# bioinfo-biols/CIRI-long

Measured on AMD Instinct MI355X. Metric: reads/s through CCS+SSW+BSJ (1/2/4/8 MI355X); % HBM roofline, higher is better.
Workload: dtype int16

## Files before the change

ciri_long_amd/csrc/ccs_poa.hip:

```cpp
#include <hip/hip_runtime.h>
#include <stdint.h>
#include "clh_device.h"
#include "clh_device_ops.h"

namespace clh {

static constexpr int CCS_K = 8;
static constexpr int CCS_DMIN = 30;
static constexpr int CCS_MIN_SUPPORT = 12;
static constexpr int CCS_SMOOTH = 3;
static constexpr int CCS_MAX_CUTS = 64;
static constexpr int CCS_MIN_TAIL = 20;
static constexpr int CCS_GUARD = 8;
static constexpr int POA_MAXP = 12;
static constexpr int POA_MAXP_ALL = 48;
static constexpr int POA_OVF_CAP = 2048;
static constexpr int POA_MAXA = 7;
static constexpr int POA_MAX_COPY = 2800;

__device__ __forceinline__ void phase_sync() {
    __syncthreads();
#ifdef POA_AGENT_PHASE_SYNC
    __builtin_amdgcn_fence(__ATOMIC_ACQUIRE, "agent");
#else
// ... 385 lines not shown
    for (int t = 1; t < CP; ++t) { runA[t] = pk_max(runA[t - 1], a[t - 1]); runB[t] = pk_max(runB[t - 1], b[t - 1]); }
    const uint32_t totA = pk_max(runA[CP - 1], a[CP - 1]), totB = pk_max(runB[CP - 1], b[CP - 1]);
    const int loA = (int)(short)(totA & 0xffffu), hiA = (int)totA >> 16, loB = (int)(short)(totB & 0xffffu), hiB = (int)totB >> 16;
    int excA = dpp_shr1(leftA, loA > hiA ? loA : hiA), excB = dpp_shr1(leftB, loB > hiB ? loB : hiB);
    wave_prefix_max2(excA, excB);
    const uint32_t exA = pack_exc(excA, totA), exB = pack_exc(excB, totB);
#pragma unroll
    for (int t = 0; t < CP; ++t) { pa[t] = pk_max(runA[t], exA); pb[t] = pk_max(runB[t], exB); }
}

__device__ __forceinline__ uint32_t pk_nz_select(uint32_t x, uint32_t d, uint32_t lo) {
    uint32_t r;
    asm("v_pk_min_u16 %0, %1, 1 op_sel_hi:[1,0]\n\tv_pk_mad_u16 %0, %0, %2, %3" : "=&v"(r) : "v"(x), "v"(d), "v"(lo));
    return r;
}
__device__ __forceinline__ uint32_t lshl_or(uint32_t a, int sh, uint32_t b) {
    uint32_t d;
    asm("v_lshl_or_b32 %0, %1, %2, %3" : "=v"(d) : "v"(a), "n"(sh), "v"(b));
    return d;
}
template <typename T>
__device__ __forceinline__ T* uniform_ptr(T* p) {
    const unsigned long long v = (unsigned long long)p;
    const uint32_t lo = (uint32_t)__builtin_amdgcn_readfirstlane((int)(uint32_t)v), hi = (uint32_t)__builtin_amdgcn_readfirstlane((int)(uint32_t)(v >> 32));
    typedef __attribute__((address_space(1))) T* gptr;
    return (T*)(gptr)(((unsigned long long)hi << 32) | lo);
}

template <int HX, int HY>
__device__ __forceinline__ uint32_t mix16(uint32_t x, uint32_t y) {
// ... 11 lines not shown
__device__ __forceinline__ void to_packed(const uint32_t (&nat)[CP], uint32_t (&p)[CP]) {
    if constexpr (CP == 1) p[0] = nat[0];
    else if constexpr (CP == 2) { p[0] = mix16<0, 0>(nat[0], nat[1]); p[1] = mix16<1, 1>(nat[0], nat[1]); }
    else if constexpr (CP == 3) { p[0] = mix16<0, 1>(nat[0], nat[1]); p[1] = mix16<1, 0>(nat[0], nat[2]); p[2] = mix16<0, 1>(nat[1], nat[2]); }
    else { p[0] = mix16<0, 0>(nat[0], nat[2]); p[1] = mix16<1, 1>(nat[0], nat[2]); p[2] = mix16<0, 0>(nat[1], nat[3]); p[3] = mix16<1, 1>(nat[1], nat[3]); }
}

static constexpr int D_F = 0x0007, D_O_SHIFT = 3, D_E_SHIFT = 8, D_Q_SHIFT = 11;
#ifndef POA_BAND_W
#define POA_BAND_W 32
#endif
static constexpr int POA_BAND = POA_BAND_W;
static constexpr int POA_H_NONE = -32768;
static constexpr int BT_MISS = -2;

template <int CP, bool SIMPLE = false>
__device__ void dp_pass_lz(const PoaWs& w, const PoaScores S, int N, int m, const int8_t* seq, int lane, const int pass, const int colbase,
                           const bool more_in, const int RING, const int slope16, int& bs_io, int& br_io, int& bc_io DBGARG)
{
    constexpr int C = 2 * CP;
    const int gp = poa_pitch(m);
    const int rmask = RING - 1;
    const bool more = SIMPLE ? false : more_in;
    const bool sw = SIMPLE ? true : (S.algorithm & 0xff) == 0, nw = SIMPLE ? false : (S.algorithm & 0xff) == 1;
    char* const gH = (char*)uniform_ptr(w.planeH);
    char* const gD = (char*)uniform_ptr(w.planeD);
    const uint2* const gri = uniform_ptr(w.ri);
    const short* const gcol0 = uniform_ptr(w.col0);
    const int cpitch = __builtin_amdgcn_readfirstlane(w.cpitch);
    const int32_t* const gorder = uniform_ptr(w.order); const int32_t* const grank = uniform_ptr(w.rank); const int32_t* const gpred = uniform_ptr(w.pred);
    const int g = S.g, e = S.e, q = S.q, c = S.c;
    const uint32_t g2 = dup16(g), e2 = dup16(e), q2 = dup16(q), c2 = dup16(c);
    const uint32_t sm2 = opaque(dup16(S.m)), dsn2 = opaque(dup16(S.n - S.m));
    const uint32_t ge2 = dup16(g - e), qc2 = dup16(q - c);
    const uint32_t NEG2 = dup16(POA_NEG), ONE2 = 0x00010001u;
    const uint32_t floor2 = sw ? 0u : 0x80008000u;
    const bool beyond_free = sw && S.n < 0 && S.g < 0 && S.q < 0;
    uint32_t* ring = poa_lds;
    const int rrow = 128 * poa_ring_cp(m);
    int* ringL = (int*)(poa_lds + RING * rrow);
    const bool last = !more;
    const int lc0 = C * lane, col0 = colbase + lc0;
    const int mc = m - 1 - colbase;
    const int lm = mc / C, tm = (mc % C) % CP, hm = (mc % C) / CP;
    uint32_t sbP[CP], jeP[CP], jcP[CP];
#pragma unroll
    for (int t = 0; t < CP; ++t) {
        const int jlo = col0 + t + 1, jhi = jlo + CP;
        sbP[t] = pack16(jlo <= m ? (int)(uint8_t)seq[jlo - 1] : 0x100, jhi <= m ? (int)(uint8_t)seq[jhi - 1] : 0x100);
        jeP[t] = pack16((lc0 + t + 1) * e, (lc0 + CP + t + 1) * e);
        jcP[t] = pack16((lc0 + t + 1) * c, (lc0 + CP + t + 1) * c);
    }
    auto row0_h = [&](int j) -> int {
        const int l1 = g + (j - 1) * e, l2 = q + (j - 1) * c;
        return (sw || j == 0) ? 0 : (l1 > l2 ? l1 : l2);
    };
    short* const gcarry = uniform_ptr(w.carry);
    const short* cprev = gcarry + (size_t)(pass & 1) * 3 * cpitch;
    short* cnext = gcarry + (size_t)((pass + 1) & 1) * 3 * cpitch;
    const bool carried = SIMPLE ? false : pass > 0;
    uint2 blk = make_uint2(0, 0); int cH = 0, cE = POA_NEG, cQ = POA_NEG;
    struct RowIn { uint2 b; int h, e, q; };
    auto fetch1 = [&](int rr) -> RowIn {
        const bool in = rr <= N;
        const int rc = in ? rr : N;
        const uint2 b = gri[rc];
        const int hc = (int)cprev[rc], ec = (int)cprev[cpitch + rc], qc = (int)cprev[2 * cpitch + rc], h0 = (int)gcol0[rc];
        RowIn x;
        x.b = in ? b : make_uint2(0, 0);
        x.h = !in ? 0 : (carried ? hc : (nw ? h0 : 0));
        x.e = in && carried ? ec : POA_NEG; x.q = in && carried ? qc : POA_NEG;
        return x;
    };
    auto fetch = [&](int rr, uint2& b, int& h, int& ee, int& qq) { const RowIn x = fetch1(rr); b = x.b; h = x.h; ee = x.e; qq = x.q; };
    auto left_of = [&](int qr) -> int { return carried ? (int)cprev[qr] : (nw ? (int)gcol0[qr] : 0); };
    fetch(1 + lane, blk, cH, cE, cQ);
    asm volatile("" :: "v"(blk.x), "v"(blk.y), "v"(cH), "v"(cE), "v"(cQ));
    uint32_t px[CP], pf[CP], po[CP];
    int pcin = 0;
#pragma unroll
    for (int t = 0; t < CP; ++t) { px[t] = 0; pf[t] = 0; po[t] = 0; }
    uint32_t bsP = sw ? 0u : 0x80008000u, brP = 0;
    uint32_t snapP[CP];
#pragma unroll
    for (int t = 0; t < CP; ++t) snapP[t] = 0;
    int nbest = -(1 << 30), nrow = 0;
    uint32_t lowP = 0x7fff7fffu;
    const bool stores = col0 + 1 <= m;
    const uint32_t lane_off = (uint32_t)(col0 + 8) * 2u;
    uint32_t beyondP[CP], endP[CP];
#pragma unroll
    for (int t = 0; t < CP; ++t) { beyondP[t] = opaque(pk_sra15(sbP[t] << 7)); endP[t] = opaque(beyond_free ? 0u : beyondP[t]); }
    for (int rb = 1; rb <= N; rb += 64) {
        uint2 nblk; int nH, nE, nQ;
        fetch(rb + 64 + lane, nblk, nH, nE, nQ);
        const int cnt = N - rb + 1 < 64 ? N - rb + 1 : 64;
        int cobH = 0, cobE = 0, cobQ = 0;
        for (int i = 0; i < cnt; ++i) {
            const int r = rb + i;
            SEC0();
            const uint32_t d0 = (uint32_t)__builtin_amdgcn_readlane((int)blk.x, i);
            int cinH = 0, cinE = POA_NEG, cinQ = POA_NEG;
            if (__builtin_expect(carried | nw, 0)) cinH = __builtin_amdgcn_readlane(cH, i);
            if (__builtin_expect(carried, 0)) { cinE = __builtin_amdgcn_readlane(cE, i); cinQ = __builtin_amdgcn_readlane(cQ, i); }
            const int vb = (int)(d0 & 0xff), np = (int)((d0 >> 8) & 0xf);
            const bool sink = (d0 & 0x1000u) != 0, tolds = (d0 & 0x4000u) != 0;
            const int p0 = (int)(d0 >> 16);
            uint32_t ss[CP];
            {
                const uint32_t vb2 = dup16(vb);
#pragma unroll
                for (int t = 0; t < CP; ++t) {
                    ss[t] = pk_nz_select(sbP[t] ^ vb2, dsn2, sm2);
                }
            }
            auto source = [&](int qr, uint32_t (&h)[CP], int& left, uint32_t (&fs)[CP], uint32_t (&os)[CP]) {
                if (qr == 0) {
#pragma unroll
                    for (int t = 0; t < CP; ++t) {
                        h[t] = pack16(row0_h(col0 + t + 1), row0_h(col0 + CP + t + 1));
                        fs[t] = pk_adds(h[t], 0xffffffffu); os[t] = fs[t];
                    }
                    left = row0_h(colbase);
                } else {
                    uint32_t dd[CP];
                    if (r - qr < RING) {
                        const uint32_t* rp = ring + (qr & rmask) * rrow + lane * CP;
#pragma unroll
                        for (int t = 0; t < CP; ++t) { h[t] = rp[t]; dd[t] = rp[64 * CP + t]; }
                        left = ringL[qr & rmask];
                    } else {
                        uint32_t nh[CP], nd[CP];
                        const uint32_t* sh = (const uint32_t*)(gH + (size_t)qr * gp * 2 + lane_off);
                        const uint32_t* sd = (const uint32_t*)(gD + (size_t)qr * gp * 2 + lane_off);
#pragma unroll
                        for (int t = 0; t < CP; ++t) {
                            nh[t] = 0; nd[t] = 0;
                            if (stores) {
                                nh[t] = __hip_atomic_load(sh + t, __ATOMIC_RELAXED, __HIP_MEMORY_SCOPE_AGENT);
                                nd[t] = __hip_atomic_load(sd + t, __ATOMIC_RELAXED, __HIP_MEMORY_SCOPE_AGENT);
                            }
                        }
                        left = left_of(qr);
                        to_packed<CP>(nh, h); to_packed<CP>(nd, dd);
                    }
#pragma unroll
                    for (int t = 0; t < CP; ++t) {
                        fs[t] = pk_adds(h[t], pk_subu(dd[t] & 0x00070007u, ONE2));
                        os[t] = pk_adds(h[t], pk_subu(pk_shr(dd[t], 3) & 0x001f001fu, ONE2));
                    }
                }
            };
            SEC(8);
            uint32_t dg[CP], MF[CP], MO[CP];
            auto one_source = [&]() {
                const uint32_t hsh0 = hand_down(px[CP - 1], pcin);
#pragma unroll
                for (int t = 0; t < CP; ++t) {
                    dg[t] = pk_adds(t == 0 ? hsh0 : px[t - 1], ss[t]);
                    MF[t] = pk_max(px[t], pf[t]); MO[t] = pk_max(px[t], po[t]);
                }
            };
            if (__builtin_expect((d0 & 0x2000u) != 0, 1)) {
                one_source();
            } else if (np <= 1) {
                source(np == 0 ? 0 : p0, px, pcin, pf, po);
                one_source();
            } else {
                const uint32_t d1 = (uint32_t)__builtin_amdgcn_readlane((int)blk.y, i);
#pragma unroll
                for (int t = 0; t < CP; ++t) { dg[t] = NEG2; MF[t] = NEG2; MO[t] = NEG2; }
                auto add_source = [&](int qr) {
                    uint32_t h[CP], fs[CP], os[CP];
                    int left = pcin;
                    if (qr == r - 1) {
#pragma unroll
                        for (int t = 0; t < CP; ++t) { h[t] = px[t]; fs[t] = pf[t]; os[t] = po[t]; }
                    } else source(qr, h, left, fs, os);
                    const uint32_t hsh0 = hand_down(h[CP - 1], left);
#pragma unroll
                    for (int t = 0; t < CP; ++t) {
                        dg[t] = pk_max(dg[t], pk_adds(t == 0 ? hsh0 : h[t - 1], ss[t]));
                        MF[t] = pk_max(MF[t], pk_max(h[t], fs[t])); MO[t] = pk_max(MO[t], pk_max(h[t], os[t]));
                    }
                };
                add_source(p0);
                add_source((int)(d1 & 0xffff));
                if (np > 2) add_source((int)(d1 >> 16));
                if (np > 3) {
                    const int vnode = __builtin_amdgcn_readfirstlane(gorder[r - 1]);
                    const int npt = np < 15 ? np : __builtin_amdgcn_readfirstlane((int)w.np[vnode]);
                    for (int s2 = 3; s2 < npt; ++s2) add_source(__builtin_amdgcn_readfirstlane(grank[poa_pred_at(w, vnode, s2)]));
                }
            }
            SEC(9);
            uint32_t M0[CP], fsn[CP], osn[CP];
#pragma unroll
            for (int t = 0; t < CP; ++t) {
                fsn[t] = pk_adds(MF[t], e2); osn[t] = pk_adds(MO[t], c2);
                M0[t] = pk_max(pk_max(dg[t], floor2), pk_max(pk_adds(MF[t], g2), pk_adds(MO[t], q2)));
            }
            uint32_t X[CP], Y[CP];
            {
                uint32_t a[CP], b[CP], pe[CP], pq[CP];
                const int leftE = cinH > cinE + e - g ? cinH : cinE + e - g;
                const int leftQ = cinH > cinQ + c - q ? cinH : cinQ + c - q;
#pragma unroll
                for (int t = 0; t < CP; ++t) { a[t] = pk_subs(M0[t], jeP[t]); b[t] = pk_subs(M0[t], jcP[t]); }
                scan_left_pk2<CP>(a, leftE, pe, b, leftQ, pq);
#pragma unroll
                for (int t = 0; t < CP; ++t) { X[t] = pk_adds(pe[t], jeP[t]); Y[t] = pk_adds(pq[t], jcP[t]); }
            }
            SEC(10);
            uint32_t Hf[CP], qhat[CP], Es[CP], D[CP];
#pragma unroll
            for (int t = 0; t < CP; ++t) { qhat[t] = pk_adds(Y[t], qc2); Hf[t] = pk_max(pk_max(M0[t], pk_adds(X[t], ge2)), qhat[t]); }
            const uint32_t q0 = hand_down(qhat[CP - 1], cinQ);
#pragma unroll
            for (int t = 0; t < CP; ++t) {
                Es[t] = pk_max(X[t], pk_adds(t == 0 ? q0 : qhat[t - 1], e2));
                const uint32_t Hm = pk_subs(Hf[t], ONE2);
                const uint32_t YF = pk_max(fsn[t], Hm), YO = pk_max(osn[t], Hm), YE = pk_max(Es[t], Hm), YQ = pk_max(Y[t], Hm);
                {
                    uint32_t dd_, t_;
                    asm("v_pk_mad_u16 %0, %2, 8, %3 op_sel_hi:[1,0,1]\n\tv_pk_mad_u16 %1, %4, 8, %5 op_sel_hi:[1,0,1]\n\t"
                        "v_pk_mad_u16 %0, %1, %6, %0\n\tv_pk_mad_u16 %0, %7, %8, %0"
                        : "=&v"(dd_), "=&v"(t_) : "v"(YO), "v"(YF), "v"(YQ), "v"(YE), "s"(0x01000100u), "v"(Hm), "s"(dup16(-2313)));
                    D[t] = dd_;
                }
            }
            SEC(11);
#pragma unroll
            for (int t = 0; t < CP; ++t) { px[t] = Hf[t]; pf[t] = fsn[t]; po[t] = osn[t]; }
            pcin = cinH;
            const int band = (slope16 && !(d0 & 0x8000u)) ? POA_BAND : (1 << 20);
            const int cen = (int)(((unsigned)r * (unsigned)slope16) >> 16);
            const bool st_row = stores && (unsigned)(col0 + C - (cen - band)) <= (unsigned)(2 * band + C - 1);
            if (__builtin_expect(st_row, 1)) {
                uint32_t nh[CP], nd[CP];
                to_natural<CP>(Hf, nh); to_natural<CP>(D, nd);
                const uint32_t voff = (uint32_t)r * (uint32_t)(gp * 2) + lane_off;
                typedef __attribute__((address_space(1))) char* gchar;
                typedef __attribute__((address_space(1))) uint32_t* gu32;
                gu32 dh = (gu32)((gchar)gH + (size_t)voff), dd = (gu32)((gchar)gD + (size_t)voff);
                typedef uint32_t u32x2 __attribute__((ext_vector_type(2)));
                typedef uint32_t u32x3 __attribute__((ext_vector_type(3)));
                typedef uint32_t u32x4 __attribute__((ext_vector_type(4)));
#ifdef POA_TEMPORAL_STORES
#define PLANE_ST(ptr, val) (*(ptr) = (val))
#else
#define PLANE_ST(ptr, val) __builtin_nontemporal_store(val, ptr)
#endif
                if constexpr (CP == 1) { PLANE_ST(dh, nh[0]); PLANE_ST(dd, nd[0]); }
                else if constexpr (CP == 2) {
                    PLANE_ST((__attribute__((address_space(1))) u32x2*)dh, (u32x2{nh[0], nh[1]})); PLANE_ST((__attribute__((address_space(1))) u32x2*)dd, (u32x2{nd[0], nd[1]}));
// ... 49 lines not shown
        asm volatile("" :: "v"(blk.x), "v"(blk.y), "v"(cH), "v"(cE), "v"(cQ));
    }
    if (more) phase_sync();
    {
        const int lo2 = (int)(short)(lowP & 0xffffu), hi2 = (int)lowP >> 16;
        if (__builtin_amdgcn_ballot_w64((lo2 < hi2 ? lo2 : hi2) <= POA_NEG)) bs_io = -(1 << 29), br_io = -1;
    }
    if (br_io < 0) return;
    {
        uint32_t bcP = 0;
#pragma unroll
        for (int t = CP - 1; t >= 0; --t) {
            const uint32_t eqm = pk_subu(pk_minu(pk_subs(bsP, snapP[t]), ONE2), ONE2);
            bcP = bfi(eqm, dup16(t), bcP);
        }
        const int vlo = (int)(short)(bsP & 0xffffu), vhi = (int)bsP >> 16;
        const int rlo = (int)(brP & 0xffffu), rhi = (int)(brP >> 16);
        const int clo = col0 + (int)(bcP & 0xffffu) + 1, chi = col0 + CP + (int)(bcP >> 16) + 1;
        int bs = vlo, br = rlo, bc = clo;
        if (vhi > vlo || (vhi == vlo && rhi < rlo)) { bs = vhi; br = rhi; bc = chi; }
        if (br == 0) bs = -(1 << 30);
#pragma unroll
        for (int d = 1; d < 64; d <<= 1) {
            const int s2 = __shfl_xor(bs, d), r2 = __shfl_xor(br, d), c2x = __shfl_xor(bc, d);
            if (s2 > bs || (s2 == bs && (r2 < br || (r2 == br && c2x < bc)))) { bs = s2; br = r2; bc = c2x; }
        }
        if (nw) { bs = nbest; br = nrow; bc = m; }
        if (br > 0 && (bs > bs_io || (bs == bs_io && br < br_io))) { bs_io = bs; br_io = br; bc_io = bc; }
    }
}

__device__ __attribute__((noinline)) void dp_rows(const PoaWs& w, const PoaScores S_, int N, int m, const int8_t* seq_, int lane, const int slope16_, int& bs_out, int& br_out, int& bc_out DBGARG)
{
    PoaScores S;
    S.algorithm = __builtin_amdgcn_readfirstlane(S_.algorithm); S.m = __builtin_amdgcn_readfirstlane(S_.m); S.n = __builtin_amdgcn_readfirstlane(S_.n);
    S.g = __builtin_amdgcn_readfirstlane(S_.g); S.e = __builtin_amdgcn_readfirstlane(S_.e); S.q = __builtin_amdgcn_readfirstlane(S_.q);
    S.c = __builtin_amdgcn_readfirstlane(S_.c); S.min_cov = 0;
    const int slope16 = __builtin_amdgcn_readfirstlane(slope16_);
    const int8_t* seq = uniform_ptr(seq_);
    constexpr int WMAX = 128 * POA_MAXCP;
    N = __builtin_amdgcn_readfirstlane(N); m = __builtin_amdgcn_readfirstlane(m);
    const int RING = poa_ring(m);
    int bs = (S.algorithm & 0xff) == 0 ? 0 : -(1 << 30), br = 0, bc = 0;
    int pass = 0;
// ... 6 lines not shown
            switch (cp) {
                case 1: dp_pass_lz<1, true>(w, S, N, m, seq, lane, pass, colbase, more, RING, slope16, bs, br, bc DBGPASS); break;
                case 2: dp_pass_lz<2, true>(w, S, N, m, seq, lane, pass, colbase, more, RING, slope16, bs, br, bc DBGPASS); break;
                default: dp_pass_lz<3, true>(w, S, N, m, seq, lane, pass, colbase, more, RING, slope16, bs, br, bc DBGPASS); break;
            }
        } else
        switch (cp) {
            case 1: dp_pass_lz<1>(w, S, N, m, seq, lane, pass, colbase, more, RING, slope16, bs, br, bc DBGPASS); break;
            case 2: dp_pass_lz<2>(w, S, N, m, seq, lane, pass, colbase, more, RING, slope16, bs, br, bc DBGPASS); break;
            case 3: dp_pass_lz<3>(w, S, N, m, seq, lane, pass, colbase, more, RING, slope16, bs, br, bc DBGPASS); break;
            default: dp_pass_lz<4>(w, S, N, m, seq, lane, pass, colbase, more, RING, slope16, bs, br, bc DBGPASS); break;
        }
        if (br < 0) break;
    }
    bs_out = bs; br_out = br; bc_out = bc;
}

static constexpr int POA_NEGW = -(1 << 29);
__host__ __device__ inline size_t poa_plane_bytes_w(int N, int m) { return (((size_t)(N + 1) * (size_t)poa_pitch(m) * 4 + 15) & ~(size_t)15) + 64; }
__host__ __device__ inline size_t poa_dp_bytes_w(int N, int m) { return poa_plane_bytes_w(N, m) + poa_plane_bytes(N, m) + 7 * (((size_t)(N + 2) * 4 + 15) & ~(size_t)15) + 64; }
struct PoaWide { int* planeH; unsigned short* planeD; int* carry; int cpitch; int* col0; };

template <int C>
__device__ void dp_pass_w(const PoaWs& w, const PoaWide& W, const PoaScores S, const int N, const int m, const int8_t* seq, const int lane, const int pass, const int colbase,
                          const bool more, int& bs_io, int& br_io, int& bc_io)
{
    const int gp = poa_pitch(m);
    const bool sw = (S.algorithm & 0xff) == 0, nw = (S.algorithm & 0xff) == 1;
    const int g = S.g, e = S.e, q = S.q, c = S.c;
    const int lc0 = C * lane, col0 = colbase + lc0;
// ... 716 lines not shown
            }
        }
        {
            const int es = hlx + ((dlx >> 8) & 7) - 1, qs = hlx + ((dlx >> 11) & 31) - 1;
            int ext;
            if (hx == es + g) ext = 1; else if (hx == hlx + g) ext = 0; else if (hx == qs + q) ext = 1; else if (hx == hlx + q) ext = 0; else return -1;
            --j;
            if (ext) { const int rc_ = left_run(); if (rc_) return rc_; }
        }
    }
    flush(j);
    return 2 * j + (moved ? 1 : 0);
}

template <bool WIDE>
__device__ __forceinline__ int poa_add(PoaWs& w, const PoaScores S, int N_, int ncap, const int8_t* seq, int m_, int lane, int* score_out, int32_t* path_out, unsigned long long* tacc, int* band_misses, const int mref)
{
    const int N = __builtin_amdgcn_readfirstlane(N_), m = __builtin_amdgcn_readfirstlane(m_);
    unsigned long long tlast = 0;
#ifdef CLH_DEBUG_POA
    tlast = __builtin_amdgcn_s_memtime();
#endif
    *score_out = 0;
    if (m == 0) return N;
    constexpr bool wide = WIDE;
    int bs = 0, br = 0, bc = 0, slope16 = 0;
    PoaWide W;
    W.planeH = nullptr; W.planeD = nullptr; W.carry = nullptr; W.cpitch = 0; W.col0 = nullptr;
    if (N > 0) {
        if (N > POA_MAX_ROWS || (S.algorithm == 1 && N > 25000)) return -1;
        const int pitch = poa_pitch(m);
// ... 39 lines not shown
                }
                f += S.e; o += S.c;
                w.score[r] = f; w.bp[r] = o;
                const int h = f > o ? f : o;
                if constexpr (WIDE) W.col0[r] = h;
                else {
                    if (h <= POA_NEG) return -4;
                    w.col0[r] = (short)h;
                }
                __syncthreads();
            }
        }
        phase_sync();
        slope16 = m > 2 * POA_BAND + 64 ? (int)(((unsigned)(mref > m ? mref : m) << 16) / (unsigned)N) : 0;
        if constexpr (WIDE) { slope16 = 0; dp_rows_w(w, W, S, N, m, seq, lane, bs, br, bc); }
        else dp_rows(w, S, N, m, seq, lane, slope16, bs, br, bc DBGPASS);
        phase_sync();
        if (br < 0) return -4;
#ifdef CLH_DEBUG_POA
        {
            constexpr int WMAX = 128 * POA_MAXCP;
            for (int cb = 0; cb < m; cb += WMAX) { const int rem = m - cb; const int cp = rem > WMAX ? POA_MAXCP : poa_cols(rem); tacc[5] += (unsigned long long)N << 4; tacc[6] += (unsigned long long)N * cp << 4; }
            tacc[7] += (unsigned long long)N * m;
        }
#endif
    }
    *score_out = bs;
    TSTAMP(0);
    bool moved = false;
    int jb = 0, je = -1;
    for (int t = lane; t < m; t += 64) w.pn[t] = 0;
    {
        int j = br > 0 ? __builtin_amdgcn_readfirstlane(bc) : 0;
        je = j - 1;
        if (br > 0) {
            phase_sync();
            BtArgs A = {w.pn, wide ? (void*)W.planeH : (void*)w.planeH, wide ? W.planeD : w.planeD, w.ri, wide ? (void*)W.col0 : (void*)w.col0, w.rank, w.pred, w.order, seq, N, m,
                        __builtin_amdgcn_readfirstlane(br), j, slope16, w.ovn, w.ovp, w.ovc, w.np};
            int rc;
            if constexpr (WIDE) rc = poa_backtrack<int, BT_W32>(A, S DBGPASS); else rc = poa_backtrack<short, BT_W>(A, S DBGPASS);
            if (!WIDE && rc == BT_MISS) {
                if (band_misses) *band_misses += 1;
                phase_sync();
                int b1 = S.algorithm == 0 ? 0 : -(1 << 30), b2 = 0, b3 = 0;
                if constexpr (!WIDE) dp_rows(w, S, N, m, seq, lane, 0, b1, b2, b3 DBGPASS);
                for (int t = lane; t < m; t += 64) w.pn[t] = 0;
                phase_sync();
                A.slope16 = 0;
                if constexpr (!WIDE) rc = poa_backtrack<short, BT_W>(A, S DBGPASS);
            }
            if (rc < 0) return -3;
            j = rc >> 1; moved = (rc & 1) != 0;
        }
        jb = S.algorithm == 1 ? 0 : j;
    }
    phase_sync();
    TSTAMP(1);
    int n = N, fail = 0;
    {
        if (N == 0 && lane == 0) { w.ovc[0] = 0; w.ovc[1] = 0; }
// ... 265 lines not shown
            const int len = cut - b;
            maxlen = len > maxlen ? len : maxlen; total += len;
            b = cut; ++nseg;
        }
        const int ncap = total + 8, mcap = maxlen + 1;
        auto to_wide_list = [&]() { if (lane == 0) { p.results[rd] = res; const int k = atomicAdd(p.wide_count, 1); p.wide_list[k] = rd; } };
        if (!WIDE && (force_wide || maxlen > POA_MAX_COPY)) { if (p.tier == 0) to_wide_list(); continue; }
        constexpr bool wide = WIDE;
        uint8_t* ws = slot;
        size_t ws_bytes = p.slot_bytes;
        int big = -1;
        const size_t need_min = poa_fixed_bytes(ncap, mcap, nullptr) + (wide ? poa_dp_bytes_w(maxlen + 8, maxlen) : poa_dp_bytes(maxlen + 8, maxlen)) + 64;
        bool use_big = need_min > p.slot_bytes;
        int N = 0, len = -1, ncols = 0;
        unsigned long long dp_cells = 0, dp_rows_n = 0;
        int band_miss_n = 0;
        for (int attempt = 0; attempt < 2; ++attempt) {
            if (use_big) {
                if (p.tier == 0 && p.n_big > 0 && need_min <= p.big_slot_bytes) {
                    if (lane == 0)
                        for (int t = 0; t < 64 && big < 0; ++t) {
                            const int cand = (int)((blockIdx.x * 7u + (unsigned)t * 131u + (unsigned)rd) % (unsigned)p.n_big);
                            if (atomicCAS(&p.big_busy[cand], 0, 1) == 0) big = cand;
                        }
                    big = __builtin_amdgcn_readfirstlane(big);
                }
                if (big < 0) { N = -2; break; }
                __builtin_amdgcn_fence(__ATOMIC_ACQUIRE, "agent");
                ws = p.big_ws + (size_t)big * p.big_slot_bytes; ws_bytes = p.big_slot_bytes;
                if (lane == 0 && p.stats) atomicAdd(p.stats, 1);
            }
            PoaWs w = carve(ws, ws_bytes, ncap, mcap);
            phase_sync();
            unsigned long long tacc[20] = {0, 0, 0, 0, 0, 0, 0, 0, 0, 0, 0, 0, 0, 0, 0, 0, 0, 0, 0, 0};
            N = 0; b = 0;
            int si = 0, mref = 0;
            for (int i = 0; i <= ncuts && N >= 0; ++i) {
                if (i == ncuts && !tail) break;
                const int cut = i < ncuts ? __builtin_amdgcn_readfirstlane(cuts[i]) : L;
                int sc1 = 0;
                if (N > 0 && cut > b) { dp_cells += (unsigned long long)N * (unsigned)(cut - b); dp_rows_n += (unsigned long long)N * (unsigned)((cut - b + 128 * POA_MAXCP - 1) / (128 * POA_MAXCP)); }
                N = poa_add<WIDE>(w, S, N, ncap, seq + b, cut - b, lane, &sc1, p.msa_col ? p.msa_col + off + b : nullptr, tacc, &band_miss_n, mref);
                mref = cut - b > mref ? cut - b : mref;
                if (p.aln_score && si < CCS_SEG_CAP && lane == 0) p.aln_score[(size_t)rd * CCS_SEG_CAP + si] = sc1;
                b = cut; ++si;
            }
            if (N == -2 && !use_big && p.tier == 0) { use_big = true; continue; }
            if (N >= 0) {
                const int mc = S.min_cov >= 0 ? S.min_cov : (nseg + 1) / 2;
#ifdef CLH_DEBUG_POA
                const unsigned long long tc0 = __builtin_amdgcn_s_memtime();
#endif
                len = poa_consensus(w, N, mc, p.ccs + off, L, lane);
#ifdef CLH_DEBUG_POA
                tacc[4] += __builtin_amdgcn_s_memtime() - tc0;
#endif
                if (len >= 0 && p.msa_col) {
// ... 16 lines not shown
            if (big >= 0) { __threadfence(); if (lane == 0) atomicExch(&p.big_busy[big], 0); }
            continue;
        }
        if (N == -2) res.status = 1;
        else if (N == -3) res.status = 5;
        else if (N == -4) res.status = 6;
        else if (N == -5) res.status = 7;
        else if (N < 0) res.status = 2;
        else if (len < 0) res.status = 3;
        else { res.nseg = nseg; res.ccs_len = len; }
        if (lane == 0) {
            p.results[rd] = res; if (p.msa_ncols) p.msa_ncols[rd] = ncols;
            if (p.stats && (WIDE || res.status != 1 || p.tier == 1 || p.n_big == 0)) {
                atomicAdd((unsigned long long*)(p.stats + 2), dp_cells); atomicAdd((unsigned long long*)(p.stats + 4), dp_rows_n);
                if (band_miss_n) atomicAdd(p.stats + 6, band_miss_n);
                if (res.status != 0) atomicAdd(p.stats + 8 + (res.status & 7), 1);
            }
        }
        __syncthreads();
        if (big >= 0) {
            __threadfence();
            if (lane == 0) atomicExch(&p.big_busy[big], 0);
        }
    }
}

__global__ void __launch_bounds__(64, POA_WAVES) poa_consensus_kernel(const CcsParams p) { poa_kernel_body<false>(p); }
__global__ void __launch_bounds__(64, 2) poa_consensus_wide_kernel(const CcsParams p) { poa_kernel_body<true>(p); }

hipError_t launch_ccs_scan(const CcsParams& p, int count, bool with_long, hipStream_t stream)
// ... 35 lines not shown
```

ciri_long_amd/csrc/clh_api.hip:

```cpp
#include <hip/hip_runtime.h>
#include <stdint.h>
#include <stdio.h>
#include <stdlib.h>
#include <string.h>

#include <algorithm>
#include <chrono>
#include <mutex>
#include <string>
#include <vector>

#include "../../include/ciri_long_hip.h"
#include "../../include/ssw_legacy.h"
#include "clh_device.h"

static thread_local std::string g_err;
static thread_local int g_code = CLH_E_ARG;
static int fail(int code, const std::string& m) { g_err = m; g_code = code; return code; }
#define HIPCHK(expr)                                                                         \
    do {                                                                                     \
        hipError_t e_ = (expr);                                                              \
        if (e_ != hipSuccess) return fail(CLH_E_HIP, std::string(#expr) + ": " + hipGetErrorString(e_)); \
    } while (0)

// ... 2446 lines not shown

extern "C" int clh_ccs_plan_stats(clh_ccs_plan* pl, int64_t* out)
{
    if (!pl || !out) return fail(CLH_E_ARG, "clh_ccs_plan_stats: null argument");
    for (int k = 0; k < 16; ++k) out[k] = 0;
    if (pl->ran && pl->n > 0) {
        HIPCHK(hipSetDevice(pl->ctx->device));
        HIPCHK(hipStreamSynchronize(pl->last_stream));
        int st[64];
        HIPCHK(hipMemcpy(st, pl->d_counter, sizeof(st), hipMemcpyDeviceToHost));
        const int* s2 = st + 2;
        out[0] = (int64_t)((unsigned long long)(unsigned)s2[2] | ((unsigned long long)(unsigned)s2[3] << 32));
        out[1] = (int64_t)((unsigned long long)(unsigned)s2[4] | ((unsigned long long)(unsigned)s2[5] << 32));
        out[2] = s2[6];
        for (int k = 1; k <= 7; ++k) out[2 + k] = s2[8 + k];
    }
    return 0;
}

extern "C" int clh_ccs_results_dev(const clh_ccs_plan* pl, const void** rows, const void** segs, const void** ccs)
{
    if (!pl) return fail(CLH_E_ARG, "clh_ccs_results_dev: null plan");
    if (rows) *rows = pl->d_res;
    if (segs) *segs = pl->d_segs;
    if (ccs) *ccs = pl->d_ccs;
    return 0;
}

extern "C" int clh_ccs_batch(clh_ctx* ctx, int32_t n, const int8_t* reads, const int64_t* read_off, clh_ccs_t* out, int32_t* segs, int8_t* ccs)
{
// ... 116 lines not shown
```

ciri_long_amd/csrc/clh_device_ops.h:

```cpp
#pragma once
#include <hip/hip_runtime.h>
#include <stdint.h>

namespace clh {
namespace {

typedef short s16x2 __attribute__((ext_vector_type(2)));
typedef unsigned short u16x2 __attribute__((ext_vector_type(2)));

__device__ __forceinline__ uint32_t pk_adds(uint32_t a, uint32_t b) { return __builtin_bit_cast(uint32_t, __builtin_elementwise_add_sat(__builtin_bit_cast(s16x2, a), __builtin_bit_cast(s16x2, b))); }
__device__ __forceinline__ uint32_t pk_subs(uint32_t a, uint32_t b) { return __builtin_bit_cast(uint32_t, __builtin_elementwise_sub_sat(__builtin_bit_cast(s16x2, a), __builtin_bit_cast(s16x2, b))); }
__device__ __forceinline__ uint32_t pk_max(uint32_t a, uint32_t b) { return __builtin_bit_cast(uint32_t, __builtin_elementwise_max(__builtin_bit_cast(s16x2, a), __builtin_bit_cast(s16x2, b))); }
__device__ __forceinline__ uint32_t pk_maxu(uint32_t a, uint32_t b) { return __builtin_bit_cast(uint32_t, __builtin_elementwise_max(__builtin_bit_cast(u16x2, a), __builtin_bit_cast(u16x2, b))); }
__device__ __forceinline__ uint32_t pk_minu(uint32_t a, uint32_t b) { return __builtin_bit_cast(uint32_t, __builtin_elementwise_min(__builtin_bit_cast(u16x2, a), __builtin_bit_cast(u16x2, b))); }
__device__ __forceinline__ uint32_t pk_subus(uint32_t a, uint32_t b) { return __builtin_bit_cast(uint32_t, __builtin_elementwise_sub_sat(__builtin_bit_cast(u16x2, a), __builtin_bit_cast(u16x2, b))); }
__device__ __forceinline__ uint32_t pk_subu(uint32_t a, uint32_t b) { return __builtin_bit_cast(uint32_t, __builtin_bit_cast(u16x2, a) - __builtin_bit_cast(u16x2, b)); }
__device__ __forceinline__ uint32_t pk_madu(uint32_t a, uint32_t b, uint32_t c) { return __builtin_bit_cast(uint32_t, __builtin_bit_cast(u16x2, a) * __builtin_bit_cast(u16x2, b) + __builtin_bit_cast(u16x2, c)); }
__device__ __forceinline__ uint32_t pk_sra15(uint32_t a) { return __builtin_bit_cast(uint32_t, __builtin_bit_cast(s16x2, a) >> (short)15); }
__device__ __forceinline__ uint32_t pk_shr(uint32_t a, int n) { return __builtin_bit_cast(uint32_t, __builtin_bit_cast(u16x2, a) >> (unsigned short)n); }
__device__ __forceinline__ uint32_t dup16(int v) { return (uint32_t)(v & 0xffff) * 0x10001u; }
__device__ __forceinline__ uint32_t pack16(int lo, int hi) { return (uint32_t)(lo & 0xffff) | ((uint32_t)hi << 16); }
__device__ __forceinline__ uint32_t bfi(uint32_t mask, uint32_t a, uint32_t b) { return (mask & a) | (~mask & b); }

__device__ __forceinline__ uint32_t opaque(uint32_t x) { asm("" : "+v"(x)); return x; }
// ... 12 lines not shown
}
__device__ __forceinline__ uint32_t bfi_keep(uint32_t mask, uint32_t a, uint32_t b) {
    uint32_t d;
    asm("v_bfi_b32 %0, %1, %2, %3" : "=v"(d) : "v"(mask), "v"(a), "v"(b));
    return d;
}
__device__ __forceinline__ uint32_t mask_keep(uint32_t x) { asm("" : "+v"(x)); return x; }
__device__ __forceinline__ uint32_t lane_is(int lane, int i) {
    uint32_t m;
    asm("v_xor_b32 %0, %2, %1\n\tv_add_u32 %0, -1, %0\n\tv_ashrrev_i32 %0, 31, %0" : "=&v"(m) : "v"(lane), "s"(i));
    return m;
}
__device__ __forceinline__ int set_lane(int v, int x, uint32_t lane_mask) { return (int)bfi_keep(lane_mask, (uint32_t)x, (uint32_t)v); }

#endif

__device__ __forceinline__ uint32_t hand_down(uint32_t v, int lane0_lo) {
    const uint32_t x = (uint32_t)__builtin_amdgcn_update_dpp((int)((uint32_t)lane0_lo << 16), (int)v, 0x138 , 0xf, 0xf, false);
    return __builtin_amdgcn_alignbit(v, x, 16);
}
__device__ __forceinline__ uint32_t hand_up(uint32_t v, int top_hi) {
    const uint32_t x = (uint32_t)__builtin_amdgcn_update_dpp((int)((uint32_t)top_hi & 0xffffu), (int)v, 0x130 , 0xf, 0xf, false);
    return __builtin_amdgcn_alignbit(x, v, 16);
}
__device__ __forceinline__ int dpp_shr1(int fill, int v) { return __builtin_amdgcn_update_dpp(fill, v, 0x138, 0xf, 0xf, false); }

__device__ __forceinline__ int wave_prefix_max(int v) {
    asm volatile("s_nop 1\n\t"
                 "v_max_i32_dpp %0, %0, %0 row_shr:1 row_mask:0xf bank_mask:0xf\n\ts_nop 1\n\t"
                 "v_max_i32_dpp %0, %0, %0 row_shr:2 row_mask:0xf bank_mask:0xf\n\ts_nop 1\n\t"
// ... 53 lines not shown
```

ciri_long_amd/hip.py:

```python
import ctypes as C
import os
import sys

import numpy as np

_HERE = os.path.dirname(os.path.abspath(__file__))
SO_PATH = os.environ.get('CLH_LIB') or os.path.join(_HERE, 'libclh.so')


class HipUnavailable(RuntimeError):
    pass


class ClhError(RuntimeError):
    pass


class AlignRow(C.Structure):
    _fields_ = [('score1', C.c_uint16), ('score2', C.c_uint16), ('ref_begin1', C.c_int32), ('ref_end1', C.c_int32),
                ('read_begin1', C.c_int32), ('read_end1', C.c_int32), ('ref_end2', C.c_int32),
                ('cigar_off', C.c_int32), ('cigar_len', C.c_int32), ('status', C.c_int32)]


ALIGN_DTYPE = np.dtype([('score1', '<u2'), ('score2', '<u2'), ('ref_begin1', '<i4'), ('ref_end1', '<i4'),
# ... 354 lines not shown
            if genmsa:
                for i in range(int(group_off[k]), int(group_off[k + 1])):
                    row = np.full(int(ncols[k]), ord('-'), dtype=np.uint8)
                    a, b = int(seq_off[i]), int(seq_off[i + 1])
                    row[col[a:b]] = seqs[a:b].view(np.uint8) if raw else bases[np.minimum(seqs[a:b], 4)]
                    rows.append(row.tobytes().decode('latin-1'))
            item = (cons, rows)
            if with_scores:
                item = item + ([int(x) for x in asc[k, :min(CCS_SEG_CAP, int(group_off[k + 1] - group_off[k]))]],)
            res.append(item)
        return res

    def poa_last_stats(self):
        out = np.zeros(16, dtype=np.int64)
        _check(lib().clh_poa_last_stats(self._h, out.ctypes.data), 'clh_poa_last_stats')
        return {'dp_cells': int(out[0]), 'dp_row_steps': int(out[1]), 'band_misses': int(out[2]), 'dropped': {k: int(out[2 + k]) for k in range(1, 8) if out[2 + k]}}

    def edit_distance_batch(self, xs, ys):
        n = len(xs)
        if n != len(ys):
            raise ValueError('edit_distance_batch: the two lists differ in length')
        ba = [x.encode() if isinstance(x, str) else bytes(x) for x in xs]
        bb = [y.encode() if isinstance(y, str) else bytes(y) for y in ys]
        a_off = np.zeros(n + 1, dtype=np.int64); b_off = np.zeros(n + 1, dtype=np.int64)
        if n:
            a_off[1:] = np.cumsum([len(x) for x in ba]); b_off[1:] = np.cumsum([len(y) for y in bb])
        a = np.frombuffer(b''.join(ba) + b'\0', dtype=np.uint8)
        b = np.frombuffer(b''.join(bb) + b'\0', dtype=np.uint8)
        out = np.zeros(n, dtype=np.int32)
        _check(lib().clh_edit_distance_batch(self._h, n, a.ctypes.data, a_off.ctypes.data, b.ctypes.data, b_off.ctypes.data, out.ctypes.data), 'clh_edit_distance_batch')
        return out
# ... 506 lines not shown
        _check(lib().clh_ccs_run(self._h, C.c_void_p(d_reads_ptr), C.c_void_p(stream)), 'clh_ccs_run')

    def timing(self):
        ms = np.zeros(2, dtype=np.float32)
        _check(lib().clh_ccs_plan_timing(self._h, ms.ctypes.data), 'clh_ccs_plan_timing')
        return float(ms[0]), float(ms[1])

    def info(self):
        out = np.zeros(6, dtype=np.int64)
        _check(lib().clh_ccs_plan_info(self._h, out.ctypes.data), 'clh_ccs_plan_info')
        return dict(zip(('slots', 'slot_bytes', 'big_slots', 'big_slot_bytes', 'ran_in_claimed_big_slot', 'ran_in_second_launch'), (int(x) for x in out)))

    def stats(self):
        out = np.zeros(16, dtype=np.int64)
        _check(lib().clh_ccs_plan_stats(self._h, out.ctypes.data), 'clh_ccs_plan_stats')
        return {'dp_cells': int(out[0]), 'dp_row_steps': int(out[1]), 'band_misses': int(out[2]), 'dropped': {k: int(out[2 + k]) for k in range(1, 8) if out[2 + k]}}

    def results_dev(self):
        a, b, c = C.c_void_p(), C.c_void_p(), C.c_void_p()
        _check(lib().clh_ccs_results_dev(self._h, C.byref(a), C.byref(b), C.byref(c)), 'clh_ccs_results_dev')
        return a.value, b.value, c.value

    def fetch(self):
        out = np.zeros(self.n, dtype=CCS_DTYPE)
        segs = np.zeros((self.n, CCS_SEG_CAP, 2), dtype=np.int32)
        ccs = np.zeros(max(1, int(self.read_off[-1])), dtype=np.int8)
        _check(lib().clh_ccs_fetch(self._h, out.ctypes.data, segs.ctypes.data, ccs.ctypes.data), 'clh_ccs_fetch')
        return out, segs, ccs


_default_ctx = {}
# ... 9 lines not shown
```

Before: 5.355 million.

## Add biased-offset POA DP pass using plain wrapping adds instead of saturating ops

Adds a biased-frame variant of the packed int16 POA row DP, used for single-pass local alignment when score magnitudes are provably bounded. Values carry a +128 bias, so saturating packed adds and subs are replaced by plain 32-bit adds that cannot overflow or cross lanes, and the match/mismatch select uses a 32-bit mad. A runtime router picks the biased path when the score parameters and length meet the bounds, otherwise the old path runs. It also adds a stats counter for biased passes, and it risks correctness if the overflow bounds are wrong.

```diff
diff --git a/ciri_long_amd/csrc/ccs_poa.hip b/ciri_long_amd/csrc/ccs_poa.hip
--- a/ciri_long_amd/csrc/ccs_poa.hip
+++ b/ciri_long_amd/csrc/ccs_poa.hip
@@ -423,6 +423,11 @@
     asm("v_pk_min_u16 %0, %1, 1 op_sel_hi:[1,0]\n\tv_pk_mad_u16 %0, %0, %2, %3" : "=&v"(r) : "v"(x), "v"(d), "v"(lo));
     return r;
 }
+__device__ __forceinline__ uint32_t pk_nz_select32(uint32_t x, int d, uint32_t lo32) {
+    uint32_t r;
+    asm("v_pk_min_u16 %0, %1, 1 op_sel_hi:[1,0]\n\tv_mad_i32_i24 %0, %0, %2, %3" : "=&v"(r) : "v"(x), "v"(d), "v"(lo32));
+    return r;
+}
 __device__ __forceinline__ uint32_t lshl_or(uint32_t a, int sh, uint32_t b) {
     uint32_t d;
     asm("v_lshl_or_b32 %0, %1, %2, %3" : "=v"(d) : "v"(a), "n"(sh), "v"(b));
@@ -464,10 +469,13 @@
 static constexpr int POA_H_NONE = -32768;
 static constexpr int BT_MISS = -2;
 
-template <int CP, bool SIMPLE = false>
+static constexpr int POA_BIAS_KMAX = 32;
+template <int CP, bool SIMPLE = false, bool BIASED = false>
 __device__ void dp_pass_lz(const PoaWs& w, const PoaScores S, int N, int m, const int8_t* seq, int lane, const int pass, const int colbase,
                            const bool more_in, const int RING, const int slope16, int& bs_io, int& br_io, int& bc_io DBGARG)
 {
+    static_assert(SIMPLE || !BIASED, "the biased frame is proved for the single-pass local form only");
+    typedef PkFrame<BIASED> F;
     constexpr int C = 2 * CP;
     const int gp = poa_pitch(m);
     const int rmask = RING - 1;
@@ -480,11 +488,12 @@
     const int cpitch = __builtin_amdgcn_readfirstlane(w.cpitch);
     const int32_t* const gorder = uniform_ptr(w.order); const int32_t* const grank = uniform_ptr(w.rank); const int32_t* const gpred = uniform_ptr(w.pred);
     const int g = S.g, e = S.e, q = S.q, c = S.c;
-    const uint32_t g2 = dup16(g), e2 = dup16(e), q2 = dup16(q), c2 = dup16(c);
-    const uint32_t sm2 = opaque(dup16(S.m)), dsn2 = opaque(dup16(S.n - S.m));
-    const uint32_t ge2 = dup16(g - e), qc2 = dup16(q - c);
-    const uint32_t NEG2 = dup16(POA_NEG), ONE2 = 0x00010001u;
-    const uint32_t floor2 = sw ? 0u : 0x80008000u;
+    const uint32_t g2 = F::konst(g), e2 = F::konst(e), q2 = F::konst(q), c2 = F::konst(c);
+    const uint32_t sm2 = opaque(F::konst(S.m)), dsn2 = opaque(BIASED ? (uint32_t)(S.n - S.m) : dup16(S.n - S.m));
+    const uint32_t ge2 = F::konst(g - e), qc2 = F::konst(q - c);
+    const uint32_t BIAS2 = dup16(F::BIAS);
+    const uint32_t NEG2 = BIASED ? 0u : dup16(POA_NEG), ONE2 = 0x00010001u;
+    const uint32_t floor2 = sw ? BIAS2 : 0x80008000u;
     const bool beyond_free = sw && S.n < 0 && S.g < 0 && S.q < 0;
     uint32_t* ring = poa_lds;
     const int rrow = 128 * poa_ring_cp(m);
@@ -498,8 +507,8 @@
     for (int t = 0; t < CP; ++t) {
         const int jlo = col0 + t + 1, jhi = jlo + CP;
         sbP[t] = pack16(jlo <= m ? (int)(uint8_t)seq[jlo - 1] : 0x100, jhi <= m ? (int)(uint8_t)seq[jhi - 1] : 0x100);
-        jeP[t] = pack16((lc0 + t + 1) * e, (lc0 + CP + t + 1) * e);
-        jcP[t] = pack16((lc0 + t + 1) * c, (lc0 + CP + t + 1) * c);
+        jeP[t] = F::offs((lc0 + t + 1) * e, (lc0 + CP + t + 1) * e);
+        jcP[t] = F::offs((lc0 + t + 1) * c, (lc0 + CP + t + 1) * c);
     }
     auto row0_h = [&](int j) -> int {
         const int l1 = g + (j - 1) * e, l2 = q + (j - 1) * c;
@@ -529,11 +538,11 @@
     uint32_t px[CP], pf[CP], po[CP];
     int pcin = 0;
 #pragma unroll
-    for (int t = 0; t < CP; ++t) { px[t] = 0; pf[t] = 0; po[t] = 0; }
-    uint32_t bsP = sw ? 0u : 0x80008000u, brP = 0;
+    for (int t = 0; t < CP; ++t) { px[t] = BIAS2; pf[t] = BIAS2; po[t] = BIAS2; }
+    uint32_t bsP = sw ? BIAS2 : 0x80008000u, brP = 0;
     uint32_t snapP[CP];
 #pragma unroll
-    for (int t = 0; t < CP; ++t) snapP[t] = 0;
+    for (int t = 0; t < CP; ++t) snapP[t] = BIAS2;
     int nbest = -(1 << 30), nrow = 0;
     uint32_t lowP = 0x7fff7fffu;
     const bool stores = col0 + 1 <= m;
@@ -561,7 +570,8 @@
                 const uint32_t vb2 = dup16(vb);
 #pragma unroll
                 for (int t = 0; t < CP; ++t) {
-                    ss[t] = pk_nz_select(sbP[t] ^ vb2, dsn2, sm2);
+                    if constexpr (BIASED) ss[t] = pk_nz_select32(sbP[t] ^ vb2, (int)dsn2, sm2);
+                    else ss[t] = pk_nz_select(sbP[t] ^ vb2, dsn2, sm2);
                 }
             }
             auto source = [&](int qr, uint32_t (&h)[CP], int& left, uint32_t (&fs)[CP], uint32_t (&os)[CP]) {
@@ -569,7 +579,8 @@
 #pragma unroll
                     for (int t = 0; t < CP; ++t) {
                         h[t] = pack16(row0_h(col0 + t + 1), row0_h(col0 + CP + t + 1));
-                        fs[t] = pk_adds(h[t], 0xffffffffu); os[t] = fs[t];
+                        if constexpr (BIASED) { h[t] += BIAS2; fs[t] = h[t] - ONE2; } else fs[t] = pk_adds(h[t], 0xffffffffu);
+                        os[t] = fs[t];
                     }
                     left = row0_h(colbase);
                 } else {
@@ -593,21 +604,30 @@
                         }
                         left = left_of(qr);
                         to_packed<CP>(nh, h); to_packed<CP>(nd, dd);
+                        if constexpr (BIASED) {
+#pragma unroll
+                            for (int t = 0; t < CP; ++t) h[t] += BIAS2;
+                        }
                     }
 #pragma unroll
                     for (int t = 0; t < CP; ++t) {
-                        fs[t] = pk_adds(h[t], pk_subu(dd[t] & 0x00070007u, ONE2));
-                        os[t] = pk_adds(h[t], pk_subu(pk_shr(dd[t], 3) & 0x001f001fu, ONE2));
+                        if constexpr (BIASED) {
+                            fs[t] = h[t] + (dd[t] & 0x00070007u) - ONE2;
+                            os[t] = h[t] + (pk_shr(dd[t], 3) & 0x001f001fu) - ONE2;
+                        } else {
+                            fs[t] = pk_adds(h[t], pk_subu(dd[t] & 0x00070007u, ONE2));
+                            os[t] = pk_adds(h[t], pk_subu(pk_shr(dd[t], 3) & 0x001f001fu, ONE2));
+                        }
                     }
                 }
             };
             SEC(8);
             uint32_t dg[CP], MF[CP], MO[CP];
             auto one_source = [&]() {
-                const uint32_t hsh0 = hand_down(px[CP - 1], pcin);
+                const uint32_t hsh0 = hand_down(px[CP - 1], pcin + F::BIAS);
 #pragma unroll
                 for (int t = 0; t < CP; ++t) {
-                    dg[t] = pk_adds(t == 0 ? hsh0 : px[t - 1], ss[t]);
+                    dg[t] = F::add(t == 0 ? hsh0 : px[t - 1], ss[t]);
                     MF[t] = pk_max(px[t], pf[t]); MO[t] = pk_max(px[t], po[t]);
                 }
             };
@@ -627,10 +647,10 @@
 #pragma unroll
                         for (int t = 0; t < CP; ++t) { h[t] = px[t]; fs[t] = pf[t]; os[t] = po[t]; }
                     } else source(qr, h, left, fs, os);
-                    const uint32_t hsh0 = hand_down(h[CP - 1], left);
+                    const uint32_t hsh0 = hand_down(h[CP - 1], left + F::BIAS);
 #pragma unroll
                     for (int t = 0; t < CP; ++t) {
-                        dg[t] = pk_max(dg[t], pk_adds(t == 0 ? hsh0 : h[t - 1], ss[t]));
+                        dg[t] = pk_max(dg[t], F::add(t == 0 ? hsh0 : h[t - 1], ss[t]));
                         MF[t] = pk_max(MF[t], pk_max(h[t], fs[t])); MO[t] = pk_max(MO[t], pk_max(h[t], os[t]));
                     }
                 };
@@ -647,8 +667,8 @@
             uint32_t M0[CP], fsn[CP], osn[CP];
 #pragma unroll
             for (int t = 0; t < CP; ++t) {
-                fsn[t] = pk_adds(MF[t], e2); osn[t] = pk_adds(MO[t], c2);
-                M0[t] = pk_max(pk_max(dg[t], floor2), pk_max(pk_adds(MF[t], g2), pk_adds(MO[t], q2)));
+                fsn[t] = F::add(MF[t], e2); osn[t] = F::add(MO[t], c2);
+                M0[t] = pk_max(pk_max(dg[t], floor2), pk_max(F::add(MF[t], g2), F::add(MO[t], q2)));
             }
             uint32_t X[CP], Y[CP];
             {
@@ -656,20 +676,20 @@
                 const int leftE = cinH > cinE + e - g ? cinH : cinE + e - g;
                 const int leftQ = cinH > cinQ + c - q ? cinH : cinQ + c - q;
 #pragma unroll
-                for (int t = 0; t < CP; ++t) { a[t] = pk_subs(M0[t], jeP[t]); b[t] = pk_subs(M0[t], jcP[t]); }
-                scan_left_pk2<CP>(a, leftE, pe, b, leftQ, pq);
-#pragma unroll
-                for (int t = 0; t < CP; ++t) { X[t] = pk_adds(pe[t], jeP[t]); Y[t] = pk_adds(pq[t], jcP[t]); }
+                for (int t = 0; t < CP; ++t) { a[t] = F::lift(M0[t], jeP[t]); b[t] = F::lift(M0[t], jcP[t]); }
+                scan_left_pk2<CP>(a, leftE + F::BIAS, pe, b, leftQ + F::BIAS, pq);
+#pragma unroll
+                for (int t = 0; t < CP; ++t) { X[t] = F::lower(pe[t], jeP[t]); Y[t] = F::lower(pq[t], jcP[t]); }
             }
             SEC(10);
             uint32_t Hf[CP], qhat[CP], Es[CP], D[CP];
 #pragma unroll
-            for (int t = 0; t < CP; ++t) { qhat[t] = pk_adds(Y[t], qc2); Hf[t] = pk_max(pk_max(M0[t], pk_adds(X[t], ge2)), qhat[t]); }
-            const uint32_t q0 = hand_down(qhat[CP - 1], cinQ);
+            for (int t = 0; t < CP; ++t) { qhat[t] = F::add(Y[t], qc2); Hf[t] = pk_max(pk_max(M0[t], F::add(X[t], ge2)), qhat[t]); }
+            const uint32_t q0 = hand_down(qhat[CP - 1], BIASED ? F::BIAS / 2 : cinQ);
 #pragma unroll
             for (int t = 0; t < CP; ++t) {
-                Es[t] = pk_max(X[t], pk_adds(t == 0 ? q0 : qhat[t - 1], e2));
-                const uint32_t Hm = pk_subs(Hf[t], ONE2);
+                Es[t] = pk_max(X[t], F::add(t == 0 ? q0 : qhat[t - 1], e2));
+                const uint32_t Hm = F::sub(Hf[t], ONE2);
                 const uint32_t YF = pk_max(fsn[t], Hm), YO = pk_max(osn[t], Hm), YE = pk_max(Es[t], Hm), YQ = pk_max(Y[t], Hm);
                 {
                     uint32_t dd_, t_;
@@ -688,7 +708,13 @@
             const bool st_row = stores && (unsigned)(col0 + C - (cen - band)) <= (unsigned)(2 * band + C - 1);
             if (__builtin_expect(st_row, 1)) {
                 uint32_t nh[CP], nd[CP];
-                to_natural<CP>(Hf, nh); to_natural<CP>(D, nd);
+                if constexpr (BIASED) {
+                    uint32_t hu[CP];
+#pragma unroll
+                    for (int t = 0; t < CP; ++t) hu[t] = Hf[t] - BIAS2;
+                    to_natural<CP>(hu, nh);
+                } else to_natural<CP>(Hf, nh);
+                to_natural<CP>(D, nd);
                 const uint32_t voff = (uint32_t)r * (uint32_t)(gp * 2) + lane_off;
                 typedef __attribute__((address_space(1))) char* gchar;
                 typedef __attribute__((address_space(1))) uint32_t* gu32;
@@ -768,7 +794,7 @@
             const uint32_t eqm = pk_subu(pk_minu(pk_subs(bsP, snapP[t]), ONE2), ONE2);
             bcP = bfi(eqm, dup16(t), bcP);
         }
-        const int vlo = (int)(short)(bsP & 0xffffu), vhi = (int)bsP >> 16;
+        const int vlo = (int)(short)(bsP & 0xffffu) - F::BIAS, vhi = ((int)bsP >> 16) - F::BIAS;
         const int rlo = (int)(brP & 0xffffu), rhi = (int)(brP >> 16);
         const int clo = col0 + (int)(bcP & 0xffffu) + 1, chi = col0 + CP + (int)(bcP >> 16) + 1;
         int bs = vlo, br = rlo, bc = clo;
@@ -782,6 +808,16 @@
         if (nw) { bs = nbest; br = nrow; bc = m; }
         if (br > 0 && (bs > bs_io || (bs == bs_io && br < br_io))) { bs_io = bs; br_io = br; bc_io = bc; }
     }
+}
+
+__device__ __forceinline__ bool poa_pass_biased(const PoaScores& S, int m) {
+#ifdef POA_PACKED_ROW_STEP
+    return false;
+#else
+    constexpr int K = POA_BIAS_KMAX, W = 128 * (POA_MAXCP < 3 ? POA_MAXCP : 3);
+    return (S.algorithm & 0xff) == 0 && m <= W && S.m >= 0 && S.m <= 32767 && S.n < 0 && S.n >= -K && S.g < 0 && S.g >= -K && S.e < 0 && S.e >= -K && S.q < 0 && S.q >= -K && S.c < 0 && S.c >= -K
+           && m * S.m <= 32767 - PkFrame<true>::BIAS - W * K - 64;
+#endif
 }
 
 __device__ __attribute__((noinline)) void dp_rows(const PoaWs& w, const PoaScores S_, int N, int m, const int8_t* seq_, int lane, const int slope16_, int& bs_out, int& br_out, int& bc_out DBGARG)
@@ -818,6 +854,36 @@
         if (br < 0) break;
     }
     bs_out = bs; br_out = br; bc_out = bc;
+}
+
+#ifndef POA_PACKED_ROW_STEP
+__device__ __attribute__((noinline)) void dp_rows_biased(const PoaWs& w, const PoaScores S_, int N, int m, const int8_t* seq_, int lane, const int slope16_, int& bs_out, int& br_out, int& bc_out DBGARG)
+{
+    PoaScores S;
+    S.algorithm = __builtin_amdgcn_readfirstlane(S_.algorithm); S.m = __builtin_amdgcn_readfirstlane(S_.m); S.n = __builtin_amdgcn_readfirstlane(S_.n);
+    S.g = __builtin_amdgcn_readfirstlane(S_.g); S.e = __builtin_amdgcn_readfirstlane(S_.e); S.q = __builtin_amdgcn_readfirstlane(S_.q);
+    S.c = __builtin_amdgcn_readfirstlane(S_.c); S.min_cov = 0;
+    const int slope16 = __builtin_amdgcn_readfirstlane(slope16_);
+    const int8_t* seq = uniform_ptr(seq_);
+    N = __builtin_amdgcn_readfirstlane(N); m = __builtin_amdgcn_readfirstlane(m);
+    const int RING = poa_ring(m);
+    int bs = 0, br = 0, bc = 0;
+    constexpr int pass = 0;
+    switch (poa_cols(m)) {
+        case 1: dp_pass_lz<1, true, true>(w, S, N, m, seq, lane, pass, 0, false, RING, slope16, bs, br, bc DBGPASS); break;
+        case 2: dp_pass_lz<2, true, true>(w, S, N, m, seq, lane, pass, 0, false, RING, slope16, bs, br, bc DBGPASS); break;
+        default: dp_pass_lz<3, true, true>(w, S, N, m, seq, lane, pass, 0, false, RING, slope16, bs, br, bc DBGPASS); break;
+    }
+    bs_out = bs; br_out = br; bc_out = bc;
+}
+#endif
+__device__ __attribute__((noinline)) bool dp_rows_routed(const PoaWs& w, const PoaScores S, int N, int m, const int8_t* seq, int lane, const int slope16, int& bs_out, int& br_out, int& bc_out DBGARG)
+{
+#ifndef POA_PACKED_ROW_STEP
+    if (poa_pass_biased(S, m)) { dp_rows_biased(w, S, N, m, seq, lane, slope16, bs_out, br_out, bc_out DBGPASS); return true; }
+#endif
+    dp_rows(w, S, N, m, seq, lane, slope16, bs_out, br_out, bc_out DBGPASS);
+    return false;
 }
 
 static constexpr int POA_NEGW = -(1 << 29);
@@ -1564,7 +1630,7 @@
 }
 
 template <bool WIDE>
-__device__ __forceinline__ int poa_add(PoaWs& w, const PoaScores S, int N_, int ncap, const int8_t* seq, int m_, int lane, int* score_out, int32_t* path_out, unsigned long long* tacc, int* band_misses, const int mref)
+__device__ __forceinline__ int poa_add(PoaWs& w, const PoaScores S, int N_, int ncap, const int8_t* seq, int m_, int lane, int* score_out, int32_t* path_out, unsigned long long* tacc, int* band_misses, int* biased_passes, const int mref)
 {
     const int N = __builtin_amdgcn_readfirstlane(N_), m = __builtin_amdgcn_readfirstlane(m_);
     unsigned long long tlast = 0;
@@ -1634,7 +1700,10 @@
         phase_sync();
         slope16 = m > 2 * POA_BAND + 64 ? (int)(((unsigned)(mref > m ? mref : m) << 16) / (unsigned)N) : 0;
         if constexpr (WIDE) { slope16 = 0; dp_rows_w(w, W, S, N, m, seq, lane, bs, br, bc); }
-        else dp_rows(w, S, N, m, seq, lane, slope16, bs, br, bc DBGPASS);
+        else {
+            const bool biased = dp_rows_routed(w, S, N, m, seq, lane, slope16, bs, br, bc DBGPASS);
+            if (biased_passes) *biased_passes += biased;
+        }
         phase_sync();
         if (br < 0) return -4;
 #ifdef CLH_DEBUG_POA
@@ -1663,7 +1732,7 @@
                 if (band_misses) *band_misses += 1;
                 phase_sync();
                 int b1 = S.algorithm == 0 ? 0 : -(1 << 30), b2 = 0, b3 = 0;
-                if constexpr (!WIDE) dp_rows(w, S, N, m, seq, lane, 0, b1, b2, b3 DBGPASS);
+                if constexpr (!WIDE) { const bool biased = dp_rows_routed(w, S, N, m, seq, lane, 0, b1, b2, b3 DBGPASS); if (biased_passes) *biased_passes += biased; }
                 for (int t = lane; t < m; t += 64) w.pn[t] = 0;
                 phase_sync();
                 A.slope16 = 0;
@@ -1959,7 +2028,7 @@
         bool use_big = need_min > p.slot_bytes;
         int N = 0, len = -1, ncols = 0;
         unsigned long long dp_cells = 0, dp_rows_n = 0;
-        int band_miss_n = 0;
+        int band_miss_n = 0, biased_n = 0;
         for (int attempt = 0; attempt < 2; ++attempt) {
             if (use_big) {
                 if (p.tier == 0 && p.n_big > 0 && need_min <= p.big_slot_bytes) {
@@ -1985,7 +2054,7 @@
                 const int cut = i < ncuts ? __builtin_amdgcn_readfirstlane(cuts[i]) : L;
                 int sc1 = 0;
                 if (N > 0 && cut > b) { dp_cells += (unsigned long long)N * (unsigned)(cut - b); dp_rows_n += (unsigned long long)N * (unsigned)((cut - b + 128 * POA_MAXCP - 1) / (128 * POA_MAXCP)); }
-                N = poa_add<WIDE>(w, S, N, ncap, seq + b, cut - b, lane, &sc1, p.msa_col ? p.msa_col + off + b : nullptr, tacc, &band_miss_n, mref);
+                N = poa_add<WIDE>(w, S, N, ncap, seq + b, cut - b, lane, &sc1, p.msa_col ? p.msa_col + off + b : nullptr, tacc, &band_miss_n, &biased_n, mref);
                 mref = cut - b > mref ? cut - b : mref;
                 if (p.aln_score && si < CCS_SEG_CAP && lane == 0) p.aln_score[(size_t)rd * CCS_SEG_CAP + si] = sc1;
                 b = cut; ++si;
@@ -2032,6 +2101,7 @@
             if (p.stats && (WIDE || res.status != 1 || p.tier == 1 || p.n_big == 0)) {
                 atomicAdd((unsigned long long*)(p.stats + 2), dp_cells); atomicAdd((unsigned long long*)(p.stats + 4), dp_rows_n);
                 if (band_miss_n) atomicAdd(p.stats + 6, band_miss_n);
+                if (biased_n) atomicAdd(p.stats + 16, biased_n);
                 if (res.status != 0) atomicAdd(p.stats + 8 + (res.status & 7), 1);
             }
         }
diff --git a/ciri_long_amd/csrc/clh_api.hip b/ciri_long_amd/csrc/clh_api.hip
--- a/ciri_long_amd/csrc/clh_api.hip
+++ b/ciri_long_amd/csrc/clh_api.hip
@@ -2484,6 +2484,7 @@
         out[1] = (int64_t)((unsigned long long)(unsigned)s2[4] | ((unsigned long long)(unsigned)s2[5] << 32));
         out[2] = s2[6];
         for (int k = 1; k <= 7; ++k) out[2 + k] = s2[8 + k];
+        out[10] = s2[16];
     }
     return 0;
 }
diff --git a/ciri_long_amd/csrc/clh_device_ops.h b/ciri_long_amd/csrc/clh_device_ops.h
--- a/ciri_long_amd/csrc/clh_device_ops.h
+++ b/ciri_long_amd/csrc/clh_device_ops.h
@@ -50,6 +50,25 @@
 __device__ __forceinline__ int set_lane(int v, int x, uint32_t lane_mask) { return (int)bfi_keep(lane_mask, (uint32_t)x, (uint32_t)v); }
 
 #endif
+
+template <bool BIASED> struct PkFrame {
+    static constexpr int BIAS = 0;
+    static __device__ __forceinline__ uint32_t konst(int k) { return dup16(k); }
+    static __device__ __forceinline__ uint32_t add(uint32_t v, uint32_t k) { return pk_adds(v, k); }
+    static __device__ __forceinline__ uint32_t sub(uint32_t v, uint32_t k) { return pk_subs(v, k); }
+    static __device__ __forceinline__ uint32_t offs(int lo, int hi) { return pack16(lo, hi); }
+    static __device__ __forceinline__ uint32_t lift(uint32_t v, uint32_t o) { return pk_subs(v, o); }
+    static __device__ __forceinline__ uint32_t lower(uint32_t v, uint32_t o) { return pk_adds(v, o); }
+};
+template <> struct PkFrame<true> {
+    static constexpr int BIAS = 128;
+    static __device__ __forceinline__ uint32_t konst(int k) { return (uint32_t)k * 0x10001u; }
+    static __device__ __forceinline__ uint32_t add(uint32_t v, uint32_t k) { return v + k; }
+    static __device__ __forceinline__ uint32_t sub(uint32_t v, uint32_t k) { return v - k; }
+    static __device__ __forceinline__ uint32_t offs(int lo, int hi) { return pack16(-lo, -hi); }
+    static __device__ __forceinline__ uint32_t lift(uint32_t v, uint32_t o) { return v + o; }
+    static __device__ __forceinline__ uint32_t lower(uint32_t v, uint32_t o) { return v - o; }
+};
 
 __device__ __forceinline__ uint32_t hand_down(uint32_t v, int lane0_lo) {
     const uint32_t x = (uint32_t)__builtin_amdgcn_update_dpp((int)((uint32_t)lane0_lo << 16), (int)v, 0x138 , 0xf, 0xf, false);
diff --git a/ciri_long_amd/hip.py b/ciri_long_amd/hip.py
--- a/ciri_long_amd/hip.py
+++ b/ciri_long_amd/hip.py
@@ -392,7 +392,8 @@
     def poa_last_stats(self):
         out = np.zeros(16, dtype=np.int64)
         _check(lib().clh_poa_last_stats(self._h, out.ctypes.data), 'clh_poa_last_stats')
-        return {'dp_cells': int(out[0]), 'dp_row_steps': int(out[1]), 'band_misses': int(out[2]), 'dropped': {k: int(out[2 + k]) for k in range(1, 8) if out[2 + k]}}
+        return {'dp_cells': int(out[0]), 'dp_row_steps': int(out[1]), 'band_misses': int(out[2]), 'biased_passes': int(out[10]),
+                'dropped': {k: int(out[2 + k]) for k in range(1, 8) if out[2 + k]}}
 
     def edit_distance_batch(self, xs, ys):
         n = len(xs)
@@ -929,7 +930,8 @@
     def stats(self):
         out = np.zeros(16, dtype=np.int64)
         _check(lib().clh_ccs_plan_stats(self._h, out.ctypes.data), 'clh_ccs_plan_stats')
-        return {'dp_cells': int(out[0]), 'dp_row_steps': int(out[1]), 'band_misses': int(out[2]), 'dropped': {k: int(out[2 + k]) for k in range(1, 8) if out[2 + k]}}
+        return {'dp_cells': int(out[0]), 'dp_row_steps': int(out[1]), 'band_misses': int(out[2]), 'biased_passes': int(out[10]),
+                'dropped': {k: int(out[2 + k]) for k in range(1, 8) if out[2 + k]}}
 
     def results_dev(self):
         a, b, c = C.c_void_p(), C.c_void_p(), C.c_void_p()
```

After: 5.268 million. 0.984x the previous value.
